# pypr/pysph

Measured on AMD Instinct MI355X. Metric: particle-updates/sec (nnps.update + AccelerationEval.compute), WCSPH 3D, fp64, higher is better.
Workload: dtype f64

## Files before the change

pysph_amd/csrc/sph_ctx.hip:

```cpp
#include <cstddef>
#include <cstdlib>
#include "sph_internal.h"

static thread_local char g_err[1024] = "";

void sph_set_error(const char *fmt, ...)
{
    va_list ap;
    va_start(ap, fmt);
    vsnprintf(g_err, sizeof g_err, fmt, ap);
    va_end(ap);
}

int DevBuf::reserve(size_t need, bool keep, hipStream_t stream)
{
    if (need <= bytes) return SPH_OK;
    size_t nb = need + need / 4 + 256;
    void *np = nullptr;
    HIP_TRY(hipMalloc(&np, nb));
    if (keep && ptr && bytes) {
        HIP_TRY(hipMemcpyAsync(np, ptr, bytes, hipMemcpyDeviceToDevice, stream));
        HIP_TRY(hipStreamSynchronize(stream));
    }
    if (ptr) (void)hipFree(ptr);
// ... 273 lines not shown
{
    SPH_TRY(sph_array_ensure_prop(c, id, prop));
    *dptr = c->arr[id].prop[prop];
    if (prop == SPH_M || prop == SPH_H) { c->arr[id].raw_hm = true; sph_mark_written(c->arr[id], prop); }
    if (prop >= SPH_R00 && prop <= SPH_R22) c->arr[id].tflag_valid = false;
    return SPH_OK;
}

int sph_set_option(sph_ctx *c, const char *key, long value)
{
    if (strcmp(key, "pair_variant") == 0) {
        if (value != 0 && value != 6) { sph_set_error("pair_variant must be 0 (direct per-lane walk) or 6 (wavefront tiles, the default)"); return SPH_ERR_ARG; }
        c->pair_variant = value;
        return SPH_OK;
    }
    if (strcmp(key, "uniform_h") == 0) { c->use_uniform_h = value; return SPH_OK; }
    if (strcmp(key, "record_f32") == 0) { c->record_f32 = value ? 1 : 0; return SPH_OK; }
    if (strcmp(key, "arith_f32") == 0) { c->arith_f32 = value ? 1 : 0; return SPH_OK; }
    if (strcmp(key, "tile_block_rows") == 0) {
        if (value < 0 || value > 4096) { sph_set_error("tile_block_rows out of range"); return SPH_ERR_ARG; }
        c->tile_block_rows = value; c->nnps_valid = false; return SPH_OK;
    }
    if (strcmp(key, "row_mod3") == 0) {
        if (value < 0 || value > 4) { sph_set_error("row_mod3 must be 0..4"); return SPH_ERR_ARG; }
        c->row_mod3 = value; return SPH_OK;
    }
    if (strcmp(key, "pack_group") == 0) { c->pack_group = value ? 1 : 0; c->pack_epoch++; return SPH_OK; }
    if (strcmp(key, "wcsph_nr") == 0) { c->wcsph_nr = value; return SPH_OK; }
    if (strcmp(key, "lds_pad") == 0) { c->lds_pad = value; return SPH_OK; }
#ifndef SPH_PROFILING
    if ((strcmp(key, "ablate") == 0 || strcmp(key, "count_iters") == 0) && value != 0) {
        sph_set_error("option '%s': this libsphhip.so was built without the pair kernel's profiling hooks (make PROFILING=1)", key);
        return SPH_ERR_ARG;
    }
#endif
    if (strcmp(key, "ablate") == 0) { c->ablate = value; return SPH_OK; }
    if (strcmp(key, "count_iters") == 0) {
        c->count_iters = value;
        if (value) { SPH_TRY(c->dbgc.reserve(64)); HIP_TRY(hipMemset(c->dbgc.ptr, 0, 64)); }
        return SPH_OK;
    }
    if (strcmp(key, "dump_counters") == 0) {
        unsigned long long h[4] = {};
        if (c->dbgc.ptr) { HIP_TRY(hipDeviceSynchronize()); HIP_TRY(hipMemcpy(h, c->dbgc.ptr, 32, hipMemcpyDeviceToHost)); }
        fprintf(stderr, "pair kernel counters: phase-2 iterations %llu, phase-2 calls %llu, wavefronts %llu, row tiles %llu\n", h[0], h[1], h[2], h[3]);
        return SPH_OK;
    }
    if (strcmp(key, "const_flags") == 0) { c->const_flags = value; return SPH_OK; }
    if (strcmp(key, "invalidate_nnps") == 0) { c->nnps_valid = false; return SPH_OK; }
    if (strcmp(key, "eos_fuse") == 0) { c->eos_fuse = value; return SPH_OK; }
    if (strcmp(key, "mass_fuse") == 0) { c->mass_fuse = value; return SPH_OK; }
    if (strcmp(key, "nl_reuse") == 0) { c->nl_reuse = value; c->nl.valid = false; return SPH_OK; }
    if (strcmp(key, "norm_masks") == 0) { c->norm_masks = value; return SPH_OK; }
    if (strcmp(key, "row_lds") == 0) { c->row_lds = value; return SPH_OK; }
    if (strcmp(key, "fill_holes") == 0) { c->fill_holes = value ? 1 : 0; return SPH_OK; }
    if (strcmp(key, "dest_list") == 0) { c->dest_list = value < 0 ? 0 : (value > 2 ? 2 : value); c->nnps_valid = false; return SPH_OK; }
    if (strcmp(key, "merge_arrays") == 0) { c->merge_arrays = value ? 1 : 0; c->nnps_valid = false; return SPH_OK; }
    if (strcmp(key, "split_pair") == 0) { c->split_pair = value ? 1 : 0; return SPH_OK; }
    if (strcmp(key, "tension_flag") == 0) { c->tension_flag = value ? 1 : 0; return SPH_OK; }
    if (strcmp(key, "lazy_tables") == 0) { c->lazy_tables = value ? 1 : 0; c->nnps_valid = false; return SPH_OK; }
    if (strcmp(key, "async_update") == 0) { c->async_update = value ? 1 : 0; return SPH_OK; }
    if (strcmp(key, "via_unordered") == 0) { c->via_unordered = value ? 1 : 0; return SPH_OK; }
    if (strcmp(key, "sort_lbits") == 0) {
        if (value != 0 && (value < 9 || value > 11)) { sph_set_error("sort_lbits must be 0 or 9..11"); return SPH_ERR_ARG; }
        c->sort_lbits = (int)value; c->hand_sort = value == 0; return SPH_OK;
    }
    sph_set_error("sph_set_option: unknown key '%s'", key);
    return SPH_ERR_ARG;
}

int sph_timer_enable(sph_ctx *c, int on) { c->timers_on = on != 0; c->timer_mask = on; return SPH_OK; }

struct AbiField { const char *st, *field; long off; };
#define ABI_F(S, F) {#S, #F, (long)offsetof(S, F)}
static const AbiField ABI_FIELDS[] = {
    ABI_F(sph_kernel, kind), ABI_F(sph_kernel, dim), ABI_F(sph_kernel, fac), ABI_F(sph_kernel, radius_scale), ABI_F(sph_kernel, deltap),
    ABI_F(sph_equation, kind), ABI_F(sph_equation, dest), ABI_F(sph_equation, nsrc), ABI_F(sph_equation, src), ABI_F(sph_equation, par),
    ABI_F(sph_group, real), ABI_F(sph_group, start_idx), ABI_F(sph_group, stop_idx), ABI_F(sph_group, neq), ABI_F(sph_group, eqs),
    ABI_F(sph_group, src_eos), ABI_F(sph_group, eos_par), ABI_F(sph_group, nl_mode), ABI_F(sph_group, phase),
    ABI_F(sph_gen_family, launch), ABI_F(sph_gen_family, dest), ABI_F(sph_gen_family, nsrc), ABI_F(sph_gen_family, src),
    ABI_F(sph_gen_family, src_flags), ABI_F(sph_gen_family, n_sprops), ABI_F(sph_gen_family, sprops), ABI_F(sph_gen_family, n_din),
    ABI_F(sph_gen_family, din), ABI_F(sph_gen_family, n_dout), ABI_F(sph_gen_family, dout), ABI_F(sph_gen_family, npar),
    ABI_F(sph_gen_family, par), ABI_F(sph_gen_family, real), ABI_F(sph_gen_family, start_idx), ABI_F(sph_gen_family, stop_idx),
    ABI_F(sph_gen_family, split_init), ABI_F(sph_gen_family, loop_all), ABI_F(sph_gen_family, also_pair), ABI_F(sph_gen_family, init_pair),
    ABI_F(sph_gen_family, nstate), ABI_F(sph_gen_family, state), ABI_F(sph_gen_family, launch_f32),
    ABI_F(sph_gen_args, stream), ABI_F(sph_gen_args, rec), ABI_F(sph_gen_args, mode), ABI_F(sph_gen_args, par), ABI_F(sph_gen_args, state),
    ABI_F(sph_gen_args, row_mod3),
};
#undef ABI_F

long sph_abi_sizeof(const char *name)
{
    if (!name) return -1;
    if (!strcmp(name, "sph_kernel")) return (long)sizeof(sph_kernel);
    if (!strcmp(name, "sph_equation")) return (long)sizeof(sph_equation);
    if (!strcmp(name, "sph_group")) return (long)sizeof(sph_group);
    if (!strcmp(name, "sph_gen_family")) return (long)sizeof(sph_gen_family);
    if (!strcmp(name, "sph_gen_args")) return (long)sizeof(sph_gen_args);
    return -1;
}

long sph_abi_offsetof(const char *name, const char *field)
{
    if (!name || !field) return -1;
    for (const AbiField &f : ABI_FIELDS)
        if (!strcmp(f.st, name) && !strcmp(f.field, field)) return f.off;
// ... 43 lines not shown
```

pysph_amd/csrc/sph_eval.hip:

```cpp
#include "sph_internal.h"
#include "sph_kernels.h"
#include "sph_pair.h"

#include <cfloat>
#include <cmath>
#include <type_traits>

struct EosArgs {
    int kind;
    double par[SPH_MAX_PAR];
    double *rho, *p, *cs;
    size_t start, stop;
    double *q[SPH_PROP_COUNT];
    uint32_t *tflag;
};

__device__ inline void jacobi_eigen3(double A[3][3], double V[3][3], double d[3])
{
    for (int i = 0; i < 3; i++) for (int j = 0; j < 3; j++) V[i][j] = (i == j) ? 1.0 : 0.0;
    for (int sweep = 0; sweep < 12; sweep++) {
        double off = fabs(A[0][1]) + fabs(A[0][2]) + fabs(A[1][2]);
        double diag = fabs(A[0][0]) + fabs(A[1][1]) + fabs(A[2][2]);
        if (off <= 1e-300 || off <= 1e-18 * diag) break;
#pragma unroll
// ... 330 lines not shown
#pragma unroll
    for (int k = 0; k < 8; k++) {
        const double *p = kernarg_read<const double *>(__builtin_offsetof(PackMArgs, prop) + ((size_t)k * SPH_MAX_ARRAYS + sl) * sizeof(double *));
        v[k] = p[o];
    }
    const double rho = v[6];
    const double q = rho != 0.0 ? v[7] * (1.0 / (rho * rho)) : 0.0;
    const double srho = ((a.cls >> sl) & 1u) ? -rho : rho;
    if (!(rho > 0.0) && fabs(v[0]) < SPH_PARKED_MIN) atomicOr(a.rho_flag, 1u);
    double hp = 0.0;
    if (VH) hp = kernarg_read<const double *>(__builtin_offsetof(PackMArgs, prop) + ((size_t)8 * SPH_MAX_ARRAYS + sl) * sizeof(double *))[o];
    a.fpos[i] = make_float4((float)(v[0] - a.gmin[0]), (float)(v[1] - a.gmin[1]), (float)(v[2] - a.gmin[2]),
                            VH ? (float)(a.hr * hp) : (float)a.hr);
    double2 pc[PACK_MAXP];
#pragma unroll
    for (int k = 0; k < PACK_MAXP; k++) pc[k] = make_double2(0.0, 0.0);
    int np;
    if (VH && F32) {
        pc[0] = __builtin_bit_cast(double2, make_float4((float)(v[0] - a.gmin[0]), (float)(v[1] - a.gmin[1]), (float)(v[2] - a.gmin[2]), (float)hp));
        pc[1] = __builtin_bit_cast(double2, make_float4((float)v[3], (float)v[4], (float)v[5], (float)srho));
        np = 2;
    } else if (VH) {
        pc[0] = make_double2(v[0], v[1]); pc[1] = make_double2(v[2], hp);
        pc[2] = make_double2(v[3], v[4]); pc[3] = make_double2(v[5], srho);
        np = 4;
    } else if (F32) {
        pc[0] = __builtin_bit_cast(double2, make_float4((float)(v[0] - a.gmin[0]), (float)(v[1] - a.gmin[1]), (float)(v[2] - a.gmin[2]), (float)v[3]));
        pc[1] = __builtin_bit_cast(double2, make_float4((float)v[4], (float)v[5], (float)srho, (float)q));
        np = 2;
    } else {
        pc[0] = make_double2(v[0], v[1]); pc[1] = make_double2(v[2], v[3]);
        pc[2] = make_double2(v[4], v[5]); pc[3] = make_double2(srho, q);
        np = 4;
    }
    emit_pieces(a, i, pc, np);
}

template <class T> struct FamWCSPH_T {
    typedef T Real;
    static constexpr uint32_t CF0 = F_CONT | F_MOM | F_XSPH;
#ifndef SPH_WCSPH_MINB
#define SPH_WCSPH_MINB 4
#endif
    static constexpr int MINB = SPH_WCSPH_MINB;
    static constexpr int NA = 8;
    static constexpr int NR = 12;
    struct Params {
        T c0, alpha, beta, gx, gy, gz, eps;
        double *arho, *au, *av, *aw, *ax, *ay, *az, *dt_cfl, *dt_force;
    };
    struct Dest {
        T u, v, w, rho, p, cs, tmpi;
        T arho, au, av, aw, ax, ay, az, dt_cfl;
    };
    template <class A> static __device__ __forceinline__ void load(Dest &D, const T *a, const A &, uint32_t)
    {
        D.u = a[0]; D.v = a[1]; D.w = a[2]; D.rho = a[4]; D.tmpi = a[5]; D.cs = a[6]; D.p = a[7];
        D.arho = D.au = D.av = D.aw = D.ax = D.ay = D.az = T(0.0);
        D.dt_cfl = T(-1.0);
    }
    static constexpr bool PRED = true;
    template <int KK, bool UH, class A>
    static __device__ __forceinline__ void pair(Dest &D, const real4<T> &pi, const real4<T> &pj, T r2,
                                                const T (&s)[NA], uint32_t fl, const A &a, bool pass = true)
    {
        PairGeomT<T> g;
        constexpr bool MRG = SPH_MERGED_RSQ && sizeof(T) == 8 && KK != 4;
        T tt_m = T(0.0);
        if constexpr (MRG) {
            if (fl & F_MOM) tt_m = pair_geom_mom<KK, UH>(g, pi, pj, r2, T(0.5) * (D.rho + s[4]), a);
            else pair_geom<KK, UH>(g, pi, pj, r2, a);
        } else {
            pair_geom<KK, UH>(g, pi, pj, r2, a);
        }
        const T tg = pair_gradfac<KK, UH>(g);
        const T vij0 = D.u - s[0], vij1 = D.v - s[1], vij2 = D.w - s[2];
        const T vdotx = vij0 * g.xij[0] + vij1 * g.xij[1] + vij2 * g.xij[2];
        const T mj = pass ? s[3] : T(0.0);
        if (fl & F_CONT) D.arho = fma(mj * tg, vdotx, D.arho);
        if (fl & (F_MOM | F_XSPH)) {
            const T rhoij = T(0.5) * (D.rho + s[4]);
            T rhoij1;
            T wij = T(0.0);
            if (fl & (F_XSPH | F_TENSILE)) wij = pair_w<KK, UH>(g);
            if (fl & F_MOM) {
                const T re = r2 + g.eps;
                const T tt = MRG ? tt_m : fast_rcp(re * rhoij);
                const T inv_re = rhoij * tt;
                rhoij1 = re * tt;
                const T hv = g.hij * vdotx;
                const T muij = raw_min(hv, T(0.0)) * inv_re;
                const T cij = T(0.5) * (D.cs + s[6]);
                const T piij = (a.p.beta * muij - a.p.alpha * cij) * muij * rhoij1;
                const T dtv = fabs(hv * (g.rinv * g.rinv));
                D.dt_cfl = raw_max(D.dt_cfl, (r2 > T(1e-12) && pass) ? dtv : T(-1.0));
                const T tmpj = s[5];
                T tmp = D.tmpi + tmpj;
                if (fl & F_TENSILE) {
                    const T qd = (a.k.deltap * g.hij) * g.h1;
                    const T wdp = SphKernel<KK>::w(qd) * g.fac;
                    T fij = wij * fast_rcp(wdp);
                    fij = fij * fij;
                    fij = fij * fij;
                    const T Ri = D.p > 0 ? T(0.01) * D.tmpi : T(0.2) * fabs(D.tmpi);
                    const T Rj = s[7] > 0 ? T(0.01) * tmpj : T(0.2) * fabs(tmpj);
                    tmp = (D.tmpi + tmpj) + (Ri + Rj) * fij;
                }
                const T ft = -mj * (tmp + piij) * tg;
                D.au = fma(ft, g.xij[0], D.au);
                D.av = fma(ft, g.xij[1], D.av);
                D.aw = fma(ft, g.xij[2], D.aw);
            } else {
                rhoij1 = fast_rcp(rhoij);
            }
            if (fl & F_XSPH) {
                const T tmp = -a.p.eps * mj * wij * rhoij1;
                D.ax = fma(tmp, vij0, D.ax);
                D.ay = fma(tmp, vij1, D.ay);
                D.az = fma(tmp, vij2, D.az);
            }
        }
    }
    template <class A> static __device__ __forceinline__ void finish(Dest &D, const A &a, uint32_t o)
    {
        if (a.dflags & F_CONT) a.p.arho[o] = D.arho;
        if (a.dflags & F_MOM) {
            T au = D.au + a.p.gx, av = D.av + a.p.gy, aw = D.aw + a.p.gz;
            a.p.au[o] = au; a.p.av[o] = av; a.p.aw[o] = aw;
            a.p.dt_cfl[o] = D.dt_cfl < T(0.0) ? T(0.0) : D.dt_cfl + a.p.c0;
            a.p.dt_force[o] = au * au + av * av + aw * aw;
        }
        if (a.dflags & F_XSPH) {
            a.p.ax[o] = D.ax + D.u; a.p.ay[o] = D.ay + D.v; a.p.az[o] = D.az + D.w;
        }
    }
};
typedef FamWCSPH_T<double> FamWCSPH;

template <class T, bool UM = false> struct FamWCSPHE_T : FamWCSPH_T<T> {
    static constexpr bool EOSF = true;
    static constexpr bool UMASS = UM;
    static constexpr int NR = 8;
    struct Raw {
        typename std::conditional<sizeof(T) == 8, double2, float4>::type q[sizeof(T) == 8 ? 4 : 2];
    };
    template <class A> static __device__ __forceinline__ void load_raw(const A &a, uint32_t jg, Raw &r)
    {
        if constexpr (sizeof(T) == 8) {
            const double2 *p = reinterpret_cast<const double2 *>(a.rec) + (unsigned long long)jg * 4;
            r.q[0] = p[0]; r.q[1] = p[1]; r.q[2] = p[2]; r.q[3] = p[3];
        } else {
            const float4 *p = reinterpret_cast<const float4 *>(a.rec) + (unsigned long long)jg * 2;
            r.q[0] = p[0]; r.q[1] = p[1];
        }
    }
    template <class A> static __device__ __forceinline__ void decode(const A &a, const Raw &r, uint32_t fl, T mu, real4<T> &pj, T (&s)[8],
                                                                     int gk = 3)
    {
        T rho;
        if constexpr (sizeof(T) == 8) {
            pj.x = r.q[0].x; pj.y = r.q[0].y; pj.z = r.q[1].x; pj.w = 0.0;
            s[0] = r.q[1].y; s[1] = r.q[2].x; s[2] = r.q[2].y; s[3] = r.q[3].y; rho = r.q[3].x;
        } else {
            pj.x = r.q[0].x; pj.y = r.q[0].y; pj.z = r.q[0].z; pj.w = 0.f;
            s[0] = r.q[0].w; s[1] = r.q[1].x; s[2] = r.q[1].y; s[3] = r.q[1].w; rho = r.q[1].z;
        }
        s[4] = rho;
        s[5] = s[6] = s[7] = T(0.0);
        if constexpr (UM) {
            const T q = s[3];
            s[3] = mu;
            if (fl & F_MOM) {
                const T ratio = rho * (T)a.e_rho01;
                s[5] = q;
                s[6] = (T)a.e_c0 * tait_cs_power(ratio, gk);
            }
        } else
        if (fl & F_MOM) {
            const T ratio = rho * (T)a.e_rho01;
            T r7, r3;
            tait_powers(ratio, gk, r7, r3);
            const T p = (T)a.e_p0 + (T)a.e_B * (r7 - T(1.0));
            s[5] = rho != T(0.0) ? p * fast_rcp(rho * rho) : T(0.0);
            s[6] = (T)a.e_c0 * r3;
            s[7] = p;
        }
    }
    template <class A> static __device__ __forceinline__ void load_fused(const A &a, uint32_t jg, uint32_t fl, T mu, real4<T> &pj, T (&s)[8])
    {
        Raw r;
        load_raw(a, jg, r);
        decode(a, r, fl, mu, pj, s);
    }
};

// ... 71 lines not shown
        const bool c1 = rho < T(0.0);
        s[3] = c1 ? -(T)a.p.mu1 : mu;
        rho = fabs(rho);
        s[4] = rho;
        const T ratio = rho * (T)a.e_rho01;
        s[5] = q;
        s[6] = (T)a.e_c0 * tait_cs_power(ratio, 3);
        s[7] = T(0.0);
    }
    template <class A> static __device__ __forceinline__ void load_fused(const A &a, uint32_t jg, uint32_t fl, T mu, real4<T> &pj, T (&s)[8])
    {
        Raw r;
        Base::load_raw(a, jg, r);
        decode(a, r, fl, mu, pj, s);
    }
    static __device__ __forceinline__ bool acts(uint32_t ct, uint32_t bit, bool dc, bool sc)
    {
        const bool c00 = ct & bit, c01 = (ct >> 4) & bit, c10 = (ct >> 8) & bit, c11 = (ct >> 12) & bit;
        return dc ? (sc ? c11 : c10) : (sc ? c01 : c00);
    }
    template <int KK, bool UH, class A>
    static __device__ __forceinline__ void pair(Dest &D, const real4<T> &pi, const real4<T> &pj, T r2,
                                                const T (&s)[8], uint32_t ct, const A &a, bool pass = true)
    {
        PairGeomT<T> g;
        constexpr bool MRG = SPH_MERGED_RSQ && sizeof(T) == 8 && KK != 4;
        T tt_m = T(0.0);
        if constexpr (MRG) tt_m = pair_geom_mom<KK, UH>(g, pi, pj, r2, T(0.5) * (D.rho + s[4]), a);
        else pair_geom<KK, UH>(g, pi, pj, r2, a);
        const T tg = pair_gradfac<KK, UH>(g);
        const T vij0 = D.u - s[0], vij1 = D.v - s[1], vij2 = D.w - s[2];
        const T vdotx = vij0 * g.xij[0] + vij1 * g.xij[1] + vij2 * g.xij[2];
        const bool sc = s[3] < T(0.0);
        const T m = fabs(s[3]);
        const bool on_c = pass && acts(ct, F_CONT, D.dc, sc), on_m = pass && acts(ct, F_MOM, D.dc, sc),
                   on_x = pass && acts(ct, F_XSPH, D.dc, sc);
        D.arho = fma((on_c ? m : T(0.0)) * tg, vdotx, D.arho);
        const T rhoij = T(0.5) * (D.rho + s[4]);
        const T wij = pair_w<KK, UH>(g);
        const T re = r2 + g.eps;
        const T tt = MRG ? tt_m : fast_rcp(re * rhoij);
        const T inv_re = rhoij * tt;
        const T rhoij1 = re * tt;
        const T hv = g.hij * vdotx;
        const T muij = raw_min(hv, T(0.0)) * inv_re;
        const T cij = T(0.5) * (D.cs + s[6]);
        const T piij = (a.p.beta * muij - a.p.alpha * cij) * muij * rhoij1;
        const T dtv = fabs(hv * (g.rinv * g.rinv));
        D.dt_cfl = raw_max(D.dt_cfl, (r2 > T(1e-12) && on_m) ? dtv : T(-1.0));
        const T ft = -(on_m ? m : T(0.0)) * ((D.tmpi + s[5]) + piij) * tg;
        D.au = fma(ft, g.xij[0], D.au);
        D.av = fma(ft, g.xij[1], D.av);
        D.aw = fma(ft, g.xij[2], D.aw);
        const T tmp = -a.p.eps * (on_x ? m : T(0.0)) * wij * rhoij1;
        D.ax = fma(tmp, vij0, D.ax);
        D.ay = fma(tmp, vij1, D.ay);
        D.az = fma(tmp, vij2, D.az);
    }
    template <class A> static __device__ __forceinline__ void finish(Dest &D, const A &a, uint32_t o, uint32_t slot)
    {
        const uint32_t ct = a.dflags;
        const uint32_t row = D.dc ? ((ct >> 8) | (ct >> 12)) & 15u : (ct | (ct >> 4)) & 15u;
        const size_t base = __builtin_offsetof(A, p) + __builtin_offsetof(Params, out) + (size_t)slot * (9 * sizeof(double *));
        auto out = [&](int k) { return kernarg_read<double *>(base + (size_t)k * sizeof(double *)); };
        if (row & F_CONT) out(0)[o] = D.arho;
        if (row & F_MOM) {
            const T au = D.au + a.p.gx, av = D.av + a.p.gy, aw = D.aw + a.p.gz;
            out(1)[o] = au; out(2)[o] = av; out(3)[o] = aw;
            out(7)[o] = D.dt_cfl < T(0.0) ? T(0.0) : D.dt_cfl + a.p.c0;
            out(8)[o] = au * au + av * av + aw * aw;
        }
        if (row & F_XSPH) {
            out(4)[o] = D.ax + D.u; out(5)[o] = D.ay + D.v; out(6)[o] = D.az + D.w;
        }
    }
};

template <class T> struct FamWCSPHMV_T : FamWCSPHM_T<T> {
    typedef FamWCSPHM_T<T> Base;
    template <class A> static __device__ __forceinline__ void load_fused(const A &a, uint32_t jg, uint32_t, T mu, real4<T> &pj, T (&s)[8])
    {
        T rho;
        if constexpr (sizeof(T) == 8) {
            const double2 *p = reinterpret_cast<const double2 *>(a.rec) + (unsigned long long)jg * 4;
            const double2 q0 = p[0], q1 = p[1], q2 = p[2], q3 = p[3];
            pj.x = q0.x; pj.y = q0.y; pj.z = q1.x; pj.w = q1.y;
            s[0] = q2.x; s[1] = q2.y; s[2] = q3.x; rho = q3.y;
        } else {
            const float4 *p = reinterpret_cast<const float4 *>(a.rec) + (unsigned long long)jg * 2;
            const float4 q0 = p[0], q1 = p[1];
            pj.x = q0.x; pj.y = q0.y; pj.z = q0.z; pj.w = q0.w;
            s[0] = q1.x; s[1] = q1.y; s[2] = q1.z; rho = q1.w;
        }
        const bool c1 = rho < T(0.0);
        s[3] = c1 ? -(T)a.p.mu1 : mu;
        rho = fabs(rho);
        s[4] = rho;
        const T ratio = rho * (T)a.e_rho01;
        T r7, r3;
        tait_powers(ratio, 3, r7, r3);
        const T p = (T)a.e_p0 + (T)a.e_B * (r7 - T(1.0));
        s[5] = rho != T(0.0) ? p * fast_rcp(rho * rho) : T(0.0);
        s[6] = (T)a.e_c0 * r3;
        s[7] = T(0.0);
    }
};

template <bool UH>
__device__ __forceinline__ void load_record_wcsph(const double *__restrict__ rj, uint32_t fl, double4 &pj, double (&s)[8])
{
    const double2 *r2 = reinterpret_cast<const double2 *>(rj);
    const double2 a0 = r2[0], a1 = r2[1], b0 = r2[2], b1 = r2[3], c = r2[4];
    pj.x = a0.x; pj.y = a0.y; pj.z = a1.x; pj.w = 0.0;
    s[0] = b0.x; s[1] = b0.y; s[2] = b1.x; s[3] = b1.y; s[4] = c.x; s[5] = c.y; s[6] = a1.y; s[7] = 0.0;
    if (!UH || (fl & F_TENSILE)) {
        const double2 d = *reinterpret_cast<const double2 *>(rj + 10);
        pj.w = d.x; s[7] = d.y;
    }
}
template <> __device__ __forceinline__ void load_record<FamWCSPH, true>(const double *__restrict__ rj, uint32_t fl, double4 &pj, double (&s)[8]) { load_record_wcsph<true>(rj, fl, pj, s); }
template <> __device__ __forceinline__ void load_record<FamWCSPH, false>(const double *__restrict__ rj, uint32_t fl, double4 &pj, double (&s)[8]) { load_record_wcsph<false>(rj, fl, pj, s); }

template <class T> struct FamDensity_T {
    typedef T Real;
    static constexpr bool PRED = true;
    static constexpr uint32_t CF0 = F_TVFSD;
    static constexpr int MINB = 4;
    static constexpr int NA = 1;
    static constexpr int NR = 6;
    struct Params { double *rho, *V; };
    struct Dest { T m, rho, V; };
    template <class A> static __device__ __forceinline__ void load(Dest &D, const T *a, const A &, uint32_t) { D.m = a[0]; D.rho = T(0.0); D.V = T(0.0); }
// ... 730 lines not shown
            if (cf == Fam::CF0) hipLaunchKernelGGL((k_pair_rowlds<Fam, K, Fam::CF0>), g1, b1, 0, c->stream, a); \
            else hipLaunchKernelGGL((k_pair_rowlds<Fam, K, 0>), g1, b1, 0, c->stream, a)
            switch (kk) {
            case 1: LAUNCHL(1); break;
            case 2: LAUNCHL(2); break;
            case 3: LAUNCHL(3); break;
            case 4: LAUNCHL(4); break;
            }
#undef LAUNCHL
            c->timers[T_N_ROWLDS].count++;
            return SPH_OK;
        }
    }
#define LAUNCHE(K)                                                                                                              \
    if (cf == Fam::CF0) hipLaunchKernelGGL((k_pair_wave<Fam, K, UHV, FP32, Fam::CF0>), g2, b2, (size_t)c->lds_pad, c->stream, a); \
    else hipLaunchKernelGGL((k_pair_wave<Fam, K, UHV, FP32, 0>), g2, b2, (size_t)c->lds_pad, c->stream, a)
    switch (kk) {
    case 1: LAUNCHE(1); break;
    case 2: LAUNCHE(2); break;
    case 3: LAUNCHE(3); break;
    case 4: LAUNCHE(4); break;
    }
#undef LAUNCHE
    return SPH_OK;
}

template <class Fam>
static void fill_common(sph_ctx *c, PairArgs<Fam> &a, const sph_kernel *K, double t)
{
    a.posh = c->posh.as<double4>();
    a.aux = c->aux.as<double>();
    a.rec = c->posh.as<double>();
    a.nrec = c->cur_nrec;
    a.fpos = c->fposb.as<float4>();
    a.dom_extent = fmax(fmax(c->xmax[0] - c->xmin[0], c->xmax[1] - c->xmin[1]), c->xmax[2] - c->xmin[2]);
    for (int k = 0; k < 3; k++) { a.nc[k] = c->nc[k]; a.xmin[k] = c->xmin[k]; }
    a.cell_size = c->cell_size;
    a.radius_scale = c->radius_scale;
    a.k.sigma = K->fac;
    a.k.deltap = K->deltap;
    a.k.dim = K->dim;
    a.t = t;
    a.dt = c->cur_dt;
    a.ablate = (int)c->ablate;
    a.dbg = c->count_iters ? c->dbgc.as<unsigned long long>() : nullptr;
    a.hu = 0.5 * (c->h_uniform + c->h_uniform);
    a.h1u = 1.0 / a.hu;
    a.facu = K->fac * a.h1u;
    if (K->dim > 1) a.facu *= a.h1u;
    if (K->dim > 2) a.facu *= a.h1u;
    a.epsu = 0.01 * a.hu * a.hu;
    a.hr2u = (c->radius_scale * c->h_uniform) * (c->radius_scale * c->h_uniform);
    a.norm_masks = (int)c->norm_masks;
    a.face_mode = 0;
    a.gfx_lo = c->gfx_lo;
    a.gfx_hi = c->gfx_hi;
}

template <class Fam> static void set_tile_order(sph_ctx *c, PairArgs<Fam> &a, const DevArray &D)
{
    a.d_tile_order = D.n_tiles ? D.tile_order.as<uint32_t>() : nullptr;
    a.row_mod3 = (int)c->row_mod3;
}
template <class Fam> static void use_dest_list(sph_ctx *c, PairArgs<Fam> &a, const DevArray &D)
{
    if (!c->dest_list || c->pair_variant != 6 || D.dlist_n == 0 || a.nl_mode || a.face_mode) return;
    a.d_list = D.dlist.as<uint32_t>();
    a.nd = (uint32_t)D.dlist_n;
    c->timers[T_N_DLIST].count++;
    a.d_tile_order = D.n_ctiles ? D.ctile_order.as<uint32_t>() : nullptr;
}

static int ensure_out(sph_ctx *c, int id, std::initializer_list<int> props)
{
    for (int p : props) SPH_TRY(sph_array_ensure_prop(c, id, p));
    return SPH_OK;
}

int nnps_csr_pair_kernel(sph_ctx *c, int src, int dst, uint32_t *count, const uint32_t *start, uint32_t *nbrs)
{
    SPH_TRY(nnps_need_tables(c));
    DevArray &S = c->arr[src], &D = c->arr[dst];
    if (D.n == 0) return SPH_OK;
    if (count && D.n > D.n_binned) HIP_TRY(hipMemsetAsync(count + D.n_binned, 0, (D.n - D.n_binned) * 4, c->stream));
    const bool uh = c->uniform_h && c->use_uniform_h;
    const bool dest_is_src = src == dst;
    const size_t total = S.n + (dest_is_src ? 0 : D.n);
    if (total >= (1ull << 32)) { sph_set_error("too many particles for 32-bit packed indices"); return SPH_ERR_ARG; }
    PackPlan pl = pack_plan(FAM_NBR);
    if (uh) pl.nr = 4;
    const bool was_f32 = c->record_f32 != 0, was_a32 = c->arith_f32 != 0;
    c->record_f32 = 0; c->arith_f32 = 0;
    c->cur_eosf = false;
    c->cur_eosv = false;
    c->cur_tvff = false;
    c->cur_elu = false;
    c->cur_umass = false;
    c->cur_nrec = pl.nr;
    int rc = c->posh.reserve((total + 64) * sizeof(double) * pl.nr);
    if (rc == SPH_OK) rc = c->aux.reserve(64);
    if (rc == SPH_OK) rc = c->fposb.reserve((total + 64) * sizeof(float4));
    for (auto &pc : c->pack_cache) pc.epoch = 0;
    if (rc == SPH_OK) rc = pack_array(c, src, 0, pl, FAM_NBR, 1u, false, true, 0);
    if (rc == SPH_OK && S.g_n > 0) rc = pack_array(c, src, 0, pl, FAM_NBR, 1u, false, true, 1);
    if (rc == SPH_OK && !dest_is_src) rc = pack_array(c, dst, S.n, pl, FAM_NBR, 1u, true, true, 0);
    c->record_f32 = was_f32; c->arith_f32 = was_a32;
// ... 851 lines not shown
```

pysph_amd/csrc/sph_internal.h:

```cpp
#pragma once

#include <hip/hip_runtime.h>

#include <cstdarg>
#include <cstdint>
#include <cstdio>
#include <cstring>
#include <string>
#include <vector>

#include "../../include/sphhip.h"

void sph_set_error(const char *fmt, ...);

#define HIP_TRY(expr)                                                              \
    do {                                                                           \
        hipError_t _e = (expr);                                                    \
        if (_e != hipSuccess) {                                                    \
            sph_set_error("%s:%d %s -> %s", __FILE__, __LINE__, #expr,             \
                          hipGetErrorString(_e));                                  \
            return SPH_ERR_HIP;                                                    \
        }                                                                          \
    } while (0)

// ... 149 lines not shown
    long async_update = 1;
    struct {
        bool valid = false;
        bool pending = false;
        int dim = 0, narrays = 0, ids[SPH_MAX_ARRAYS] = {};
        double radius_scale = 0, cell_size_in = 0, extend[3] = {}, hr[2] = {};
    } lag;
    long park_cells = 0;
    DevBuf dom_counts;
    double *dom_pin = nullptr;
    hipEvent_t dom_ev = nullptr;
    bool dom_queued = false;
    hipEvent_t lag_ev = nullptr;
    double *pin_async = nullptr;
    GridHost rep;
    bool rep_valid = false;
    long n_async_updates = 0;

    DevBuf cub_tmp, red_part, red_out, posh, aux, fposb, dkeys, dperm, tmp_u32a, tmp_u32b, gen_state, gapq;
    double *pinned = nullptr;

    long pair_variant = 6;
    long ablate = 0;
    long count_iters = 0;
    DevBuf dbgc;
    long const_flags = 1;
    long use_uniform_h = 1;
    long arith_f32 = 0;
    long record_f32 = 0;
    long tile_block_rows = 8;
    long row_mod3 = 3;
    double cur_dt = 0.0;
    DevBuf csr_start[SPH_MAX_ARRAYS], csr_nbrs[SPH_MAX_ARRAYS];
    unsigned long long pack_epoch = 0;
    long pack_group = 0;
    PackCache pack_cache[SPH_MAX_ARRAYS];
    long wcsph_nr = 0;
    long lds_pad = 0;
    int cur_nrec = 0;
    bool cur_eosf = false;
    bool cur_umass = false;
    bool cur_eosv = false;
    bool cur_elu = false;
    bool cur_tvff = false;
    long mass_fuse = 1;
    bool want_mrange = false;
    long block_sorted_outputs = 0;
    long eos_fuse = 1;
    long nl_reuse = 0;
    long fill_holes = 1;
    long row_lds = 0;
    long dest_list = 1;
    long norm_masks = 1;
    DevBuf nlbuf;
    struct { bool valid = false; unsigned long long epoch = 0; int dst = -1, src = -1; size_t start = 0, stop = 0, nd = 0; } nl;
    unsigned long long nnps_epoch = 0;
    double h_known[2] = {0.0, -1.0};

    DevBuf interp_vol[SPH_MAX_ARRAYS], interp_vol1[SPH_MAX_ARRAYS], interp_rho[SPH_MAX_ARRAYS],
           interp_mom, interp_out;
    struct { bool valid = false; unsigned long long epoch = 0; int dest = -1, nsrc = 0, srcs[SPH_MAX_ARRAYS] = {}, kind = 0, dim = 0;
             double fac = 0; size_t nd = 0; unsigned hm_writes = 0; } interp_mc;

    void *comm = nullptr;

    bool timers_on = false;
    int timer_mask = 1;
    Timer timers[T_COUNT];
};

struct ScopedTimer {
    sph_ctx *c;
    int key;
    hipEvent_t a = nullptr, b = nullptr;
    ScopedTimer(sph_ctx *ctx, int k);
    ~ScopedTimer();
};

int nnps_minmax(sph_ctx *c, int narrays, const int *ids, double *out8, int mm);
int dev_scan_u32(sph_ctx *c, const uint32_t *in, uint32_t *out, size_t n, bool exclusive);
int dev_scan_u64(sph_ctx *c, const unsigned long long *in, unsigned long long *out, size_t n, bool exclusive);
int nnps_need_tables(sph_ctx *c);
int nnps_build_csr_device(sph_ctx *c, int src, int dst, DevBuf &start, DevBuf &nbrs, size_t *total);
int nnps_csr_pair_kernel(sph_ctx *c, int src, int dst, uint32_t *count, const uint32_t *start, uint32_t *nbrs);

static inline unsigned div_up(size_t a, unsigned b) { return (unsigned)((a + b - 1) / b); }
```

pysph_amd/csrc/sph_pair.h:

```cpp
#pragma once

#include <hip/hip_runtime.h>
#include <cstdint>

#include "sphhip.h"
#include "sph_kernels.h"

template <class T> __device__ __forceinline__ T r2_exact(T dx, T dy, T dz)
{
#pragma clang fp contract(off)
    const T a = dx * dx, b = dy * dy, c = dz * dz;
    return (a + b) + c;
}

template <class T> struct Real4Of;
template <> struct Real4Of<double> { typedef double4 type; };
template <> struct Real4Of<float> { typedef float4 type; };
template <class T> using real4 = typename Real4Of<T>::type;


struct KernelConst {
    double sigma;
    double deltap;
    int dim;
// ... 11 lines not shown

static __host__ __device__ inline int tait_gk(double gamma)
{
    return gamma == 7.0 ? 3 : gamma == 5.0 ? 2 : gamma == 3.0 ? 1 : gamma == 1.0 ? 0 : -1;
}
template <class T> __device__ __forceinline__ T tait_cs_power(T ratio, int gk)
{
    if (gk == 3) return (ratio * ratio) * ratio;
    if (gk == 2) return ratio * ratio;
    return gk == 1 ? ratio : T(1.0);
}
template <class T> __device__ __forceinline__ void tait_powers(T ratio, int gk, T &rg, T &rk)
{
    const T r2 = ratio * ratio;
    if (gk == 3) { rk = r2 * ratio; rg = (r2 * r2) * rk; }
    else if (gk == 2) { rk = r2; rg = (r2 * r2) * ratio; }
    else if (gk == 1) { rk = ratio; rg = r2 * ratio; }
    else { rk = T(1.0); rg = ratio; }
}

template <class Fam> struct PairArgs {
    int nsrc;
    SrcDesc src[SPH_MAX_ARRAYS];
    const double4 *posh;
    const double *aux;
    const double *rec;
    int nrec;
    const float4 *fpos;
    double dom_extent;
    uint32_t d_off, nd;
    double d_mu;
    const uint32_t *d_keys, *d_fkeys, *d_perm;
    const uint8_t *d_slot;
    const uint32_t *d_tile_order;
    const uint32_t *d_list;
    int face_mode, gfx_lo, gfx_hi;
    int row_mod3;
    uint32_t d_start, d_stop;
    int nc[3];
    double xmin[3];
    double cell_size;
    double radius_scale;
    KernelConst k;
    uint32_t dflags;
    unsigned long long *dbg;
    int ablate;
    int skip_init;
    int skip_post;
    double t, dt;
    double hu, h1u, facu, epsu, hr2u;
    uint32_t *nl;
    int nl_mode;
    int norm_masks;
    double e_rho01, e_c0, e_B, e_p0;
    int e_gk;
    typename Fam::Params p;
};

template <class F, class = void> struct fam_merged { static constexpr bool value = false; };
template <class F> struct fam_merged<F, decltype((void)F::MERGED)> { static constexpr bool value = F::MERGED; };

template <class V> __device__ __forceinline__ V kernarg_read(size_t byte_offset)
{
    typedef const char __attribute__((address_space(4))) *kptr;
    const kptr ka = (kptr)__builtin_amdgcn_kernarg_segment_ptr();
    return *reinterpret_cast<const V __attribute__((address_space(4))) *>(ka + byte_offset);
}

template <class F, class = void> struct fam_token { static constexpr bool value = false; };
template <class F> struct fam_token<F, decltype((void)F::TOKEN)> { static constexpr bool value = F::TOKEN; };

template <class F, class = void> struct fam_eosf { static constexpr bool value = false; };
template <class F> struct fam_eosf<F, decltype((void)F::EOSF)> { static constexpr bool value = F::EOSF; };


#ifndef SPH_NEWTON_STEPS
#define SPH_NEWTON_STEPS 1
#endif
__device__ __forceinline__ double fast_rcp(double d)
{
    double x = __builtin_amdgcn_rcp(d);
    double e = fma(-d, x, 1.0);
    x = fma(x, e, x);
    if (SPH_NEWTON_STEPS > 1) {
        e = fma(-d, x, 1.0);
        x = fma(x, e, x);
    }
    return x;
}
__device__ __forceinline__ void fast_sqrt_rsqrt(double a, double &s, double &rs)
{
    a = raw_max(a, 1e-300);
    double y = __builtin_amdgcn_rsq(a);
    double g = a * y, h = 0.5 * y;
    double r = fma(-h, g, 0.5);
    g = fma(g, r, g);
    h = fma(h, r, h);
    if (SPH_NEWTON_STEPS > 1) {
        r = fma(-h, g, 0.5);
        g = fma(g, r, g);
        h = fma(h, r, h);
    }
    s = g;
    rs = h + h;
}
__device__ __forceinline__ float fast_rcp(float d) { return __builtin_amdgcn_rcpf(d); }
__device__ __forceinline__ void fast_sqrt_rsqrt(float a, float &s, float &rs)
{
    a = fmaxf(a, 1e-35f);
    rs = __builtin_amdgcn_rsqf(a);
    s = a * rs;
}

template <class T> struct PairGeomT {
    T xij[3];
    T r2, rij, rinv, hij, h1, q, fac, eps;
};
typedef PairGeomT<double> PairGeom;

template <int KK, bool UH, class T, class A>
// ... 165 lines not shown
    const uint32_t wt = xcd_tile(blockIdx.x, gridDim.x) * WPB + (uint32_t)wv;
    uint32_t dtile = wt >> 2;
    if (dtile * 256u >= a.nd) return;
    if (a.d_tile_order) dtile = a.d_tile_order[dtile];
    const uint32_t tbase = dtile * 256u + (wt & 3u) * 64u;
    const uint32_t i = tbase + t;
    if (tbase >= a.nd) return;
    const bool valid = i < a.nd;
    uint32_t ic = valid ? i : a.nd - 1;
    if (a.d_list) ic = a.d_list[ic];
    const uint32_t o = a.d_perm[ic];
    uint32_t slot = 0;
    bool active;
    if constexpr (fam_merged<Fam>::value) {
        slot = a.d_slot[ic];
        const unsigned long long rg = kernarg_read<unsigned long long>(__builtin_offsetof(PairArgs<Fam>, p) + Fam::rng_offset(slot));
        active = valid && o >= (uint32_t)rg && o < (uint32_t)(rg >> 32);
    } else {
        active = valid && o >= a.d_start && o < a.d_stop;
    }
    const uint32_t fkey = a.d_fkeys[ic];
    const uint32_t key = fkey / SPH_NSUB;
    const int ncx = a.nc[0], ncy = a.nc[1], ncz = a.nc[2];
    const int row = key / ncx;
    const int cx = (int)(key % ncx) * SPH_NSUB + (int)(fkey % SPH_NSUB);
    bool facew = true;
    if (a.face_mode != 0 || a.gfx_lo > -0x7fffffff || a.gfx_hi < 0x7fffffff) {
        int mn = active ? cx : 0x7fffffff, mx = active ? cx : -0x7fffffff;
#pragma unroll
        for (int o = 32; o > 0; o >>= 1) { mn = min(mn, __shfl_xor(mn, o, 64)); mx = max(mx, __shfl_xor(mx, o, 64)); }
        mn = __builtin_amdgcn_readfirstlane(mn); mx = __builtin_amdgcn_readfirstlane(mx);
        facew = mn <= mx && (mn - XWIN <= a.gfx_lo || mx + XWIN >= a.gfx_hi);
        if (mn > mx && !a.nl_mode) return;
        if (a.face_mode == 1 && facew) return;
        if (a.face_mode == 2 && !facew) return;
    }
    real4<T> pi;
    typename Fam::Dest D;
    uint32_t wtok = 0;
    if constexpr (fam_token<Fam>::value) wtok = Fam::wave_token(a);
    T cur_mu = (T)a.d_mu;
    auto fetch = [&](uint32_t jg, uint32_t flags, real4<T> &pj, T (&sj)[Fam::NA]) {
        if constexpr (fam_token<Fam>::value) Fam::load_fused(a, jg, flags, cur_mu, pj, sj, wtok);
        else if constexpr (fam_eosf<Fam>::value) Fam::load_fused(a, jg, flags, cur_mu, pj, sj);
        else if constexpr (F32) load_record_f32<Fam, T>(reinterpret_cast<const float *>(a.rec) + (unsigned long long)jg * NR, pj, sj);
        else load_record<Fam, UH>(a.rec + (unsigned long long)jg * NR, flags, pj, sj);
    };
    {
        T sd_[Fam::NA];
        fetch(a.d_off + ic, a.dflags, pi, sd_);
        if (UH) pi.w = (T)a.hu;
        if constexpr (fam_merged<Fam>::value) Fam::load(D, sd_, a, o, slot);
        else Fam::load(D, sd_, a, o);
    }
    const int nfx = ncx * SPH_NSUB;
    const T hi_r = (T)a.radius_scale * pi.w;
    const T hi2 = UH ? (T)a.hr2u : hi_r * hi_r;
    const int row_first = __builtin_amdgcn_readfirstlane(row), row_last = __builtin_amdgcn_readlane(row, 63);
    if (DBGC(a) && t == 0) atomicAdd(DBGC(a) + 2, 1ull);

    auto do_pair = [&](uint32_t jg, uint32_t flags) {
        real4<T> pj;
        T sj[Fam::NA];
        fetch(jg, flags, pj, sj);
        pin_record<Fam::NA, T>(pj, sj);
        T hj2 = hi2;
        if (!UH) { hj2 = (T)a.radius_scale * pj.w; hj2 *= hj2; }
        const T r2 = r2_exact<T>(pi.x - pj.x, pi.y - pj.y, pi.z - pj.z);
        if (((r2 < hi2) || (r2 < hj2)) && ABLATE(a) != 1) Fam::template pair<KK, UH>(D, pi, pj, r2, sj, flags, a);
    };

    int cq = 0;
    auto phase2 = [&](uint32_t flags) {
        unsigned long long m = 0;
        uint32_t jb = 0;
        int q = 0;
        if (cq > 0 && ABLATE(a) != 2) { m = smask[0][t]; jb = sjb[0][t]; }
        const uint32_t self = a.d_off + ic;
        if (__any(m != 0)) {
            if (DBGC(a) && t == 0) atomicAdd(DBGC(a) + 1, 1ull);
            do {
                if (DBGC(a) && t == 0) atomicAdd(DBGC(a), 1ull);
                const bool has = m != 0;
                uint32_t j = has ? jb + (uint32_t)__builtin_ctzll(m) : self;
                m &= m - 1;
                if (m == 0 && q + 1 < cq) { ++q; m = smask[q][t]; jb = sjb[q][t]; }
                if (ABLATE(a) == 3) j = self;
                if constexpr (Fam::PRED) {
                    real4<T> pj;
                    T sj[Fam::NA];
                    fetch(j, flags, pj, sj);
                    T hj2 = hi2;
                    if (!UH) { hj2 = (T)a.radius_scale * pj.w; hj2 *= hj2; }
                    const T r2 = r2_exact<T>(pi.x - pj.x, pi.y - pj.y, pi.z - pj.z);
                    const bool pass = has && ((r2 < hi2) || (r2 < hj2)) && ABLATE(a) != 1;
                    Fam::template pair<KK, UH>(D, pi, pj, r2, sj, flags, a, pass);
                } else {
                    if (has) do_pair(j, flags);
                }
            } while (__any(m != 0));
        }
        cq = 0;
    };

    uint32_t *const nlw = a.nl_mode ? a.nl + (size_t)wt * NLW : nullptr;
    bool reuse = false, unsaved = false;
    if (a.nl_mode == 2) {
        const uint32_t nq = nlw[t];
        reuse = !__any(nq == NL_NONE);
        if (reuse) {
            const uint32_t off0 = a.src[0].off;
            const int nqmax = wave_max_i32((int)nq);
            for (int q = 0; q < nqmax; q++) {
                const uint32_t *w = nlw + 64 * (1 + 3 * q) + t;
                smask[q][t] = (unsigned long long)w[0] | ((unsigned long long)w[64] << 32);
                sjb[q][t] = w[128] + off0;
            }
            __builtin_amdgcn_fence(__ATOMIC_ACQ_REL, "wavefront");
            cq = active ? (int)nq : 0;
        }
    }

    for (int s = 0; s < a.nsrc; s++) {
    const SrcDesc sd = a.src[s];
    if (sd.ghost && !facew) continue;
    const uint32_t fl = CF ? CF : sd.flags;
    cur_mu = (T)sd.mu;
    int R = row_first, st = 0, part_resume = 0;
    uint32_t tb_resume = 0;
    bool resumed = false;
    for (;;) {
    bool more = false;
    for (; R <= row_last && !more && !reuse && ABLATE(a) != 6; R++, st = 0) {
        const bool inseg = active && row == R;
        const unsigned long long segm = __ballot(inseg);
        if (!segm) continue;
        const int cxa = __builtin_amdgcn_readlane(cx, __builtin_ctzll(segm));
        const int cxb = __builtin_amdgcn_readlane(cx, 63 - __builtin_clzll(segm));
        const int cyR = R % ncy, czR = R / ncy;
        const int xa = max(cxa - XWIN, 0), xb = min(cxb + XWIN, nfx - 1);
        const int ncs = xb - xa + 2;
        const double binw = a.cell_size * (1.0 / SPH_NSUB);
        const float oxf = (float)(binw * xa);
        const float oyf = (float)(a.cell_size * (cyR - 1));
        const float ozf = (float)(a.cell_size * (czR - 1));
        const double L = fmax(a.cell_size * (double)max((xb - xa) / SPH_NSUB + 2, 4), a.dom_extent);
        const float slack = (float)(L * 1.5e-6);
        const float4 fpi = a.fpos[a.d_off + ic];
        const float fxs = fpi.x - oxf, fys = fpi.y - oyf, fzs = fpi.z - ozf;
        const f2 fx = {fxs, fxs}, fy = {fys, fys}, fz = {fzs, fzs};
        const float hif = (float)hi_r * 1.000001f + prefilter_slack(fpi, slack, (float)a.dom_extent);
        const float hi2f = hif * hif;
        const int mycl = max(cx - XWIN, xa) - xa, mych = min(cx + XWIN, xb) + 1 - xa;

        for (; st < 9; st++) {
            const int st2 = a.row_mod3 == 4 ? (st + (int)(wt % 9u)) % 9 : st;
            const int sy = st2 % 3 - 1, sz = st2 / 3 - 1;
            const int dy = (a.row_mod3 & 1) ? (sy + 1 - cyR % 3 + 4) % 3 - 1 : sy;
            const int dz = (a.row_mod3 & 2) ? (sz + 1 - czR % 3 + 4) % 3 - 1 : sz;
            const int yy = cyR + dy, zz = czR + dz;
            if (yy < 0 || yy >= ncy || zz < 0 || zz >= ncz) continue;
            const uint32_t rowb = (uint32_t)(ncx * (yy + ncy * zz)) * SPH_NSUB;
            const uint32_t j0 = sd.fine_start[rowb + xa], j1 = sd.fine_start[rowb + xb + 1];
            const bool csl_ok = ncs <= WCSL && j1 - j0 < 65536u;
            uint32_t tb = j0;
            int part = 0;
            if (resumed) { tb = tb_resume; part = part_resume; resumed = false; }
            const bool csl_now = tb != j0;
            for (; tb < j1; tb += WCAP, part = 0) {
                const int tn = (int)min((uint32_t)WCAP, j1 - tb);
                if (DBGC(a) && t == 0) atomicAdd(DBGC(a) + 3, 1ull);
                if (csl_ok && (tb == j0 || csl_now))
                    for (int q = t; q < ncs; q += 64) csl[q] = (unsigned short)(sd.fine_start[rowb + xa + q] - j0);
                for (int k = t; k < tn + 8; k += 64) {
                    float vx = 3.0e18f, vy = 3.0e18f, vz = 3.0e18f, vw = 0.f;
                    if (k < tn) {
                        const float4 fj = a.fpos[sd.off + tb + k];
                        vx = fj.x - oxf; vy = fj.y - oyf; vz = fj.z - ozf;
                        const float hjf = fj.w * 1.000001f + (UH ? slack : prefilter_slack(fj, slack, (float)a.dom_extent));
                        vw = hjf * hjf;
// ... 1 lines not shown
                    tx[k] = vx; ty[k] = vy; tz[k] = vz;
                    if (!UH) tw[k] = vw;
                }
                __builtin_amdgcn_fence(__ATOMIC_ACQ_REL, "wavefront");
                int s0 = 0, len = 0;
                if (inseg) {
                    int lo, hi;
                    if (csl_ok) { lo = (int)(j0 + csl[mycl] - tb); hi = (int)(j0 + csl[mych] - tb); }
                    else { lo = (int)(sd.fine_start[rowb + xa + mycl] - tb); hi = (int)(sd.fine_start[rowb + xa + mych] - tb); }
                    lo = max(lo, 0); hi = min(hi, tn);
                    s0 = lo & ~1;
                    len = hi - s0;
                }
                for (;; part++) {
                    const int plen = len - AMAXLEN * part;
                    const int ps0 = plen > 0 ? s0 + AMAXLEN * part : 0;
                    if (part > 0 && !__any(plen > 0)) break;
                    const int lenc = ABLATE(a) == 7 ? 0 : min(plen, AMAXLEN);
                    uint32_t wd[3] = {0u, 0u, 0u};
#pragma unroll
                    for (int gw = 0; gw < 3; gw++) {
                        if (!__any(32 * gw < lenc)) break;
                        uint32_t mm = 0;
                        int g8 = 0;
                        for (; g8 < 4 && __any(32 * gw + 8 * g8 < lenc); g8++) {
                            const float *tb0 = tile + (ps0 + 32 * gw + 8 * g8);
#pragma unroll
                            for (int p = 0; p < 4; p++) {
                                const f2 X = *reinterpret_cast<const f2 *>(tb0 + 2 * p);
                                const f2 Y = *reinterpret_cast<const f2 *>(tb0 + TS + 2 * p);
                                const f2 Z = *reinterpret_cast<const f2 *>(tb0 + 2 * TS + 2 * p);
                                const f2 ex = fx - X, ey = fy - Y, ez = fz - Z;
                                f2 nthr = {-hi2f, -hi2f};
                                if (!UH) {
                                    const f2 W = *reinterpret_cast<const f2 *>(tb0 + 3 * TS + 2 * p);
                                    nthr.x = -fmaxf(hi2f, W.x);
                                    nthr.y = -fmaxf(hi2f, W.y);
                                }
                                f2 d = __builtin_elementwise_fma(ex, ex, nthr);
                                d = __builtin_elementwise_fma(ey, ey, d);
                                d = __builtin_elementwise_fma(ez, ez, d);
                                mm = __builtin_amdgcn_alignbit(mm, __float_as_uint(d.x), 31);
                                mm = __builtin_amdgcn_alignbit(mm, __float_as_uint(d.y), 31);
                            }
                        }
                        if (g8 < 4) mm <<= 8 * (4 - g8);
                        mm = __builtin_bitreverse32(mm);
                        const int rem = lenc - 32 * gw;
                        wd[gw] = rem >= 32 ? mm : (rem > 0 ? (mm & ((1u << rem) - 1u)) : 0u);
                    }
                    unsigned long long m0 = (unsigned long long)wd[0] | ((unsigned long long)wd[1] << 32);
                    uint32_t m2 = wd[2];
                    uint32_t jb0 = sd.off + tb + (uint32_t)ps0;
                    if (a.norm_masks && __any(m2 != 0)) {
                        const int sh = m0 ? __builtin_ctzll(m0) : (m2 ? 64 + __builtin_ctz(m2) : 0);
                        if (sh >= 64) { m0 = (unsigned long long)(m2 >> (sh - 64)); m2 = 0; }
                        else if (sh > 0) {
                            m0 = (m0 >> sh) | ((unsigned long long)m2 << (64 - sh));
                            m2 = sh >= 32 ? 0u : (m2 >> sh);
                        }
                        jb0 += (uint32_t)sh;
                    }
                    if (__any(cq + (m0 != 0) + (m2 != 0) > WLQ)) { more = true; break; }
                    if (m0) { smask[cq][t] = m0; sjb[cq][t] = jb0; cq++; }
                    if (m2) { smask[cq][t] = m2; sjb[cq][t] = jb0 + 64u; cq++; }
                }
                __builtin_amdgcn_fence(__ATOMIC_ACQ_REL, "wavefront");
                if (more) { tb_resume = tb; part_resume = part; break; }
            }
            if (more) break;
        }
        if (more) break;
    }
    if (a.nl_mode == 1 && s == 0) {
        if (unsaved || more) nlw[t] = NL_NONE;
        else {
            __builtin_amdgcn_fence(__ATOMIC_ACQ_REL, "wavefront");
            nlw[t] = (uint32_t)cq;
            const int nqmax = wave_max_i32(cq);
            for (int q = 0; q < nqmax; q++) {
                uint32_t *w = nlw + 64 * (1 + 3 * q) + t;
                const unsigned long long m = q < cq ? smask[q][t] : 0ull;
                w[0] = (uint32_t)m; w[64] = (uint32_t)(m >> 32);
                w[128] = q < cq ? sjb[q][t] - sd.off : 0u;
            }
        }
    }
    phase2(fl);
    if (!more) break;
    unsaved = true;
    resumed = true;
    }
    }
    if (active) {
        if constexpr (fam_merged<Fam>::value) Fam::finish(D, a, o, slot);
        else Fam::finish(D, a, o);
    }
}


template <class F, class = void> struct fam_rowlds { static constexpr bool value = false; };
template <class F> struct fam_rowlds<F, decltype((void)F::ROWLDS)> { static constexpr bool value = F::ROWLDS; };

#ifndef SPH_WCAP_L
#define SPH_WCAP_L 96
#endif
// ... 168 lines not shown
```

Before: 1.954 billion.

## Skip self-pair in WCSPH masks and prefetch next neighbor slot ahead

```diff
diff --git a/pysph_amd/csrc/sph_ctx.hip b/pysph_amd/csrc/sph_ctx.hip
--- a/pysph_amd/csrc/sph_ctx.hip
+++ b/pysph_amd/csrc/sph_ctx.hip
@@ -349,6 +349,7 @@
     if (strcmp(key, "mass_fuse") == 0) { c->mass_fuse = value; return SPH_OK; }
     if (strcmp(key, "nl_reuse") == 0) { c->nl_reuse = value; c->nl.valid = false; return SPH_OK; }
     if (strcmp(key, "norm_masks") == 0) { c->norm_masks = value; return SPH_OK; }
+    if (strcmp(key, "skip_self") == 0) { c->skip_self = value ? 1 : 0; return SPH_OK; }
     if (strcmp(key, "row_lds") == 0) { c->row_lds = value; return SPH_OK; }
     if (strcmp(key, "fill_holes") == 0) { c->fill_holes = value ? 1 : 0; return SPH_OK; }
     if (strcmp(key, "dest_list") == 0) { c->dest_list = value < 0 ? 0 : (value > 2 ? 2 : value); c->nnps_valid = false; return SPH_OK; }
diff --git a/pysph_amd/csrc/sph_eval.hip b/pysph_amd/csrc/sph_eval.hip
--- a/pysph_amd/csrc/sph_eval.hip
+++ b/pysph_amd/csrc/sph_eval.hip
@@ -406,14 +406,17 @@
     struct Dest {
         T u, v, w, rho, p, cs, tmpi;
         T arho, au, av, aw, ax, ay, az, dt_cfl;
+        T xeps;
     };
-    template <class A> static __device__ __forceinline__ void load(Dest &D, const T *a, const A &, uint32_t)
+    template <class A> static __device__ __forceinline__ void load(Dest &D, const T *a, const A &a_, uint32_t)
     {
         D.u = a[0]; D.v = a[1]; D.w = a[2]; D.rho = a[4]; D.tmpi = a[5]; D.cs = a[6]; D.p = a[7];
         D.arho = D.au = D.av = D.aw = D.ax = D.ay = D.az = T(0.0);
         D.dt_cfl = T(-1.0);
+        D.xeps = a_.p.eps;
     }
     static constexpr bool PRED = true;
+    static constexpr bool SELF_ZERO = true;
     template <int KK, bool UH, class A>
     static __device__ __forceinline__ void pair(Dest &D, const real4<T> &pi, const real4<T> &pj, T r2,
                                                 const T (&s)[NA], uint32_t fl, const A &a, bool pass = true)
@@ -468,7 +471,7 @@
                 rhoij1 = fast_rcp(rhoij);
             }
             if (fl & F_XSPH) {
-                const T tmp = -a.p.eps * mj * wij * rhoij1;
+                const T tmp = -D.xeps * mj * wij * rhoij1;
                 D.ax = fma(tmp, vij0, D.ax);
                 D.ay = fma(tmp, vij1, D.ay);
                 D.az = fma(tmp, vij2, D.az);
@@ -495,6 +498,8 @@
     static constexpr bool EOSF = true;
     static constexpr bool UMASS = UM;
     static constexpr int NR = 8;
+    static constexpr bool SLOT_AHEAD = true;
+    static __device__ __forceinline__ void pin_loop_constants(typename FamWCSPH_T<T>::Dest &D) { asm volatile("" : "+v"(D.xeps)); }
     struct Raw {
         typename std::conditional<sizeof(T) == 8, double2, float4>::type q[sizeof(T) == 8 ? 4 : 2];
     };
@@ -672,7 +677,7 @@
         D.au = fma(ft, g.xij[0], D.au);
         D.av = fma(ft, g.xij[1], D.av);
         D.aw = fma(ft, g.xij[2], D.aw);
-        const T tmp = -a.p.eps * (on_x ? m : T(0.0)) * wij * rhoij1;
+        const T tmp = -D.xeps * (on_x ? m : T(0.0)) * wij * rhoij1;
         D.ax = fma(tmp, vij0, D.ax);
         D.ay = fma(tmp, vij1, D.ay);
         D.az = fma(tmp, vij2, D.az);
@@ -698,6 +703,7 @@
 
 template <class T> struct FamWCSPHMV_T : FamWCSPHM_T<T> {
     typedef FamWCSPHM_T<T> Base;
+    static constexpr bool SLOT_AHEAD = false;
     template <class A> static __device__ __forceinline__ void load_fused(const A &a, uint32_t jg, uint32_t, T mu, real4<T> &pj, T (&s)[8])
     {
         T rho;
@@ -1534,6 +1540,7 @@
     a.epsu = 0.01 * a.hu * a.hu;
     a.hr2u = (c->radius_scale * c->h_uniform) * (c->radius_scale * c->h_uniform);
     a.norm_masks = (int)c->norm_masks;
+    a.skip_self = (int)c->skip_self;
     a.face_mode = 0;
     a.gfx_lo = c->gfx_lo;
     a.gfx_hi = c->gfx_hi;
diff --git a/pysph_amd/csrc/sph_internal.h b/pysph_amd/csrc/sph_internal.h
--- a/pysph_amd/csrc/sph_internal.h
+++ b/pysph_amd/csrc/sph_internal.h
@@ -225,6 +225,7 @@
     long row_lds = 0;
     long dest_list = 1;
     long norm_masks = 1;
+    long skip_self = 1;
     DevBuf nlbuf;
     struct { bool valid = false; unsigned long long epoch = 0; int dst = -1, src = -1; size_t start = 0, stop = 0, nd = 0; } nl;
     unsigned long long nnps_epoch = 0;
diff --git a/pysph_amd/csrc/sph_pair.h b/pysph_amd/csrc/sph_pair.h
--- a/pysph_amd/csrc/sph_pair.h
+++ b/pysph_amd/csrc/sph_pair.h
@@ -87,6 +87,8 @@
     uint32_t *nl;
     int nl_mode;
     int norm_masks;
+    int skip_self;
+    int pad_;
     double e_rho01, e_c0, e_B, e_p0;
     int e_gk;
     typename Fam::Params p;
@@ -101,6 +103,12 @@
     const kptr ka = (kptr)__builtin_amdgcn_kernarg_segment_ptr();
     return *reinterpret_cast<const V __attribute__((address_space(4))) *>(ka + byte_offset);
 }
+
+template <class F, class = void> struct fam_selfzero { static constexpr bool value = false; };
+template <class F> struct fam_selfzero<F, decltype((void)F::SELF_ZERO)> { static constexpr bool value = F::SELF_ZERO; };
+
+template <class F, class = void> struct fam_slot_ahead { static constexpr bool value = false; };
+template <class F> struct fam_slot_ahead<F, decltype((void)F::SLOT_AHEAD)> { static constexpr bool value = F::SLOT_AHEAD; };
 
 template <class F, class = void> struct fam_token { static constexpr bool value = false; };
 template <class F> struct fam_token<F, decltype((void)F::TOKEN)> { static constexpr bool value = F::TOKEN; };
@@ -372,6 +380,7 @@
         if (UH) pi.w = (T)a.hu;
         if constexpr (fam_merged<Fam>::value) Fam::load(D, sd_, a, o, slot);
         else Fam::load(D, sd_, a, o);
+        if constexpr (fam_slot_ahead<Fam>::value) Fam::pin_loop_constants(D);
     }
     const int nfx = ncx * SPH_NSUB;
     const T hi_r = (T)a.radius_scale * pi.w;
@@ -391,6 +400,8 @@
     };
 
     int cq = 0;
+    uint32_t skiprec = 0xFFFFFFFFu;
+    if constexpr (fam_selfzero<Fam>::value) { if (a.skip_self && !a.nl_mode) skiprec = a.d_off + ic; }
     auto phase2 = [&](uint32_t flags) {
         unsigned long long m = 0;
         uint32_t jb = 0;
@@ -403,9 +414,17 @@
                 if (DBGC(a) && t == 0) atomicAdd(DBGC(a), 1ull);
                 const bool has = m != 0;
                 uint32_t j = has ? jb + (uint32_t)__builtin_ctzll(m) : self;
-                m &= m - 1;
-                if (m == 0 && q + 1 < cq) { ++q; m = smask[q][t]; jb = sjb[q][t]; }
                 if (ABLATE(a) == 3) j = self;
+                constexpr bool AHEAD = Fam::PRED && fam_slot_ahead<Fam>::value;
+                unsigned long long nm = 0;
+                uint32_t njb = 0;
+                if constexpr (AHEAD) {
+                    const int qn = min(q + 1, WLQ - 1);
+                    nm = smask[qn][t]; njb = sjb[qn][t];
+                } else {
+                    m &= m - 1;
+                    if (m == 0 && q + 1 < cq) { ++q; m = smask[q][t]; jb = sjb[q][t]; }
+                }
                 if constexpr (Fam::PRED) {
                     real4<T> pj;
                     T sj[Fam::NA];
@@ -417,6 +436,14 @@
                     Fam::template pair<KK, UH>(D, pi, pj, r2, sj, flags, a, pass);
                 } else {
                     if (has) do_pair(j, flags);
+                }
+                if constexpr (AHEAD) {
+                    __builtin_amdgcn_sched_barrier(0);
+                    m &= m - 1;
+                    const bool adv = m == 0 && q + 1 < cq;
+                    m = adv ? nm : m;
+                    jb = adv ? njb : jb;
+                    q = adv ? q + 1 : q;
                 }
             } while (__any(m != 0));
         }
@@ -446,6 +473,7 @@
     if (sd.ghost && !facew) continue;
     const uint32_t fl = CF ? CF : sd.flags;
     cur_mu = (T)sd.mu;
+    if constexpr (fam_slot_ahead<Fam>::value) asm volatile("" : "+v"(cur_mu));
     int R = row_first, st = 0, part_resume = 0;
     uint32_t tb_resume = 0;
     bool resumed = false;
@@ -553,6 +581,11 @@
                     unsigned long long m0 = (unsigned long long)wd[0] | ((unsigned long long)wd[1] << 32);
                     uint32_t m2 = wd[2];
                     uint32_t jb0 = sd.off + tb + (uint32_t)ps0;
+                    if constexpr (fam_selfzero<Fam>::value) {
+                        const uint32_t ds = skiprec - jb0;
+                        if (ds < 64u) m0 &= ~(1ull << ds);
+                        else if (ds < 96u) m2 &= ~(1u << (ds - 64u));
+                    }
                     if (a.norm_masks && __any(m2 != 0)) {
                         const int sh = m0 ? __builtin_ctzll(m0) : (m2 ? 64 + __builtin_ctz(m2) : 0);
                         if (sh >= 64) { m0 = (unsigned long long)(m2 >> (sh - 64)); m2 = 0; }
```

Measured after the change: 1.945 billion. No clear change (-0.5%).
